# wjmaddox/online_gp

Hardware: AMD Instinct MI355X
Metric: streaming updates/sec (WISKI, 50^3 inducing grid) (higher is better)
Workload: dtype f32

## Files before the change

include/wiski.h:

```cpp
#ifndef WISKI_H
#define WISKI_H

#include <stdint.h>

#ifdef __cplusplus
extern "C" {
#endif

#define WISKI_OK 0
#define WISKI_E_BADARG (-1)
#define WISKI_E_LAUNCH (-2)
#define WISKI_E_WORKSPACE (-3)
#define WISKI_E_NOTCONV (-4)
#define WISKI_PENDING 1

#define WISKI_MAX_DIM 4

typedef struct wiski_grid {
  int32_t d;
  int32_t g[WISKI_MAX_DIM];
  double g0[WISKI_MAX_DIM];
  double h[WISKI_MAX_DIM];
} wiski_grid;

// ... 68 lines not shown
int64_t wiski_pcg_workspace_bytes(const wiski_grid* grid, int32_t k, int32_t max_iter, int32_t elem_size);
int wiski_pcg_f32(const wiski_grid* grid, const float* d_A_st, const float* d_tcol, float kscale, const float* d_evec, const float* d_evec2, const float* d_eval, float shift, const float* d_RHS, int32_t k, float* d_U, float* d_Z, int32_t warm, double tol, int32_t max_iter, int32_t check_every, int32_t first_check, void* d_work, int64_t work_bytes, int32_t* h_iters, double* h_relres, const int32_t* d_err, int32_t* h_err, int32_t a_sym, float* d_R, void* stream);
int wiski_pcg_f64(const wiski_grid* grid, const double* d_A_st, const double* d_tcol, double kscale, const double* d_evec, const double* d_evec2, const double* d_eval, double shift, const double* d_RHS, int32_t k, double* d_U, double* d_Z, int32_t warm, double tol, int32_t max_iter, int32_t check_every, int32_t first_check, void* d_work, int64_t work_bytes, int32_t* h_iters, double* h_relres, const int32_t* d_err, int32_t* h_err, int32_t a_sym, double* d_R, void* stream);

typedef int (*wiski_allreduce_fn)(void* ctx, void* d_vec, int64_t n_vec, int32_t elem_bytes, double* d_dots, int64_t n_dots, void* stream);
typedef struct wiski_shard {
  int32_t rank, nranks;
  void* comm;
  wiski_allreduce_fn allreduce;
  void* ctx;
} wiski_shard;
int wiski_shard_groups(int32_t d, int32_t rank, int32_t nranks, int32_t* g_lo, int32_t* g_hi);

typedef struct wiski_twolevel {
  int32_t r;
  int32_t nslab;
  const uint64_t* d_mask;
  const int32_t* d_off;
  const uint16_t* d_pos;
  const float* d_N;
  uint64_t* d_cs;
  float* d_mc;
  int32_t mc_cols;
} wiski_twolevel;

typedef struct wiski_pcg_async {
  int32_t state;
  int32_t it;
  int64_t seq;
  void* poll;
  int32_t prezeroed;
  int32_t guard_ok;
  double shift;
} wiski_pcg_async;
int wiski_pcg_async_f32(const wiski_grid* grid, const float* d_A_st, const float* d_tcol, float kscale, const float* d_evec, const float* d_evec2, const float* d_eval, float shift, const float* d_RHS, int32_t k, float* d_U, float* d_Z, int32_t warm, double tol, int32_t max_iter, int32_t check_every, int32_t first_check, void* d_work, int64_t work_bytes, int32_t* h_iters, double* h_relres, const int32_t* d_err, int32_t* h_err, int32_t a_sym, float* d_R, void* stream, wiski_pcg_async* handle, int32_t mode);
int wiski_pcg_async_f64(const wiski_grid* grid, const double* d_A_st, const double* d_tcol, double kscale, const double* d_evec, const double* d_evec2, const double* d_eval, double shift, const double* d_RHS, int32_t k, double* d_U, double* d_Z, int32_t warm, double tol, int32_t max_iter, int32_t check_every, int32_t first_check, void* d_work, int64_t work_bytes, int32_t* h_iters, double* h_relres, const int32_t* d_err, int32_t* h_err, int32_t a_sym, double* d_R, void* stream, wiski_pcg_async* handle, int32_t mode);
int wiski_pcg_async_free(wiski_pcg_async* handle);
int wiski_pcg_async_guard(const wiski_pcg_async* handle, const void** d_guard, int64_t* expect);
int wiski_pcg_zero_regions_f32(const wiski_grid* grid, int32_t k, int32_t max_iter, void* d_work, int32_t a_sym, void** p1, int64_t* n1_bytes, void** p2, int64_t* n2_bytes);
int wiski_pcg_zero_regions_f64(const wiski_grid* grid, int32_t k, int32_t max_iter, void* d_work, int32_t a_sym, void** p1, int64_t* n1_bytes, void** p2, int64_t* n2_bytes);
int64_t wiski_scatter_bin_bytes(const wiski_grid* grid, int64_t n, int32_t elem_size);
int wiski_scatter_stats_step_f32(const wiski_grid* grid, const float* d_x, const float* d_y, const float* d_wa, const float* d_wb, const float* d_noise, int64_t n, float* d_b, float* d_A_half, float* d_cnt, const float* d_u, float* d_res, float* d_mean_out, double* d_stats, int32_t* d_err, void* z1, int64_t n1_bytes, void* z2, int64_t n2_bytes, const void* d_guard, int64_t guard_expect, void* d_bin, int64_t bin_bytes, void* stream);
int wiski_scatter_stats_step_f64(const wiski_grid* grid, const double* d_x, const double* d_y, const double* d_wa, const double* d_wb, const double* d_noise, int64_t n, double* d_b, double* d_A_half, double* d_cnt, const double* d_u, double* d_res, double* d_mean_out, double* d_stats, int32_t* d_err, void* z1, int64_t n1_bytes, void* z2, int64_t n2_bytes, const void* d_guard, int64_t guard_expect, void* d_bin, int64_t bin_bytes, void* stream);
int wiski_gather_zero_f32(const wiski_grid* grid, const float* d_x, int64_t n, const float* d_V, int32_t k, float* d_out, int32_t* d_err, void* z1, int64_t n1_bytes, void* z2, int64_t n2_bytes, int32_t* zeroed, void* stream);
int wiski_gather_zero_f64(const wiski_grid* grid, const double* d_x, int64_t n, const double* d_V, int32_t k, double* d_out, int32_t* d_err, void* z1, int64_t n1_bytes, void* z2, int64_t n2_bytes, int32_t* zeroed, void* stream);

typedef struct wiski_stream_args_f32 {
  float* d_A_half; float* d_b; float* d_cnt; double* d_stats; int32_t* d_err;
  float* d_U; float* d_Z; float* d_R;
  const float* d_tcol; float kscale; const float* d_evec; const float* d_evec2; const float* d_eval; float shift;
  double tol; int32_t max_iter; int32_t check_every; void* d_work; int64_t work_bytes;
  void* d_bin; int64_t bin_bytes;
  const wiski_shard* shard;
  const wiski_twolevel* two_level;
  int32_t keep[3];
} wiski_stream_args_f32;
typedef struct wiski_stream_args_f64 {
  double* d_A_half; double* d_b; double* d_cnt; double* d_stats; int32_t* d_err;
  double* d_U; double* d_Z; double* d_R;
  const double* d_tcol; double kscale; const double* d_evec; const double* d_evec2; const double* d_eval; double shift;
  double tol; int32_t max_iter; int32_t check_every; void* d_work; int64_t work_bytes;
  void* d_bin; int64_t bin_bytes;
  const wiski_shard* shard;
  const wiski_twolevel* two_level;
  int32_t keep[3];
} wiski_stream_args_f64;
// ... 194 lines not shown
```

online_gp_amd/csrc/pcg.h:

```cpp
#pragma once
#include "wiski_common.h"

template <typename real>
struct PcgArgs {
  const real* A = nullptr;
  bool a_sym = false;
  const real* RHS = nullptr;
  int k = 0;
  const real* tcol = nullptr;
  real kscale = (real)0;
  const real* evec = nullptr;
  const real* evec2 = nullptr;
  const real* eval = nullptr;
  real shift = (real)0;
  const wiski_twolevel* two_level = nullptr;
  int keep[3] = {0, 0, 0};
  real* U = nullptr;
  real* Z = nullptr;
  real* R = nullptr;
  int warm = 0;
  double tol = 0;
  int max_iter = 0;
  int check_every = 0;
  int first_check = 0;
  void* work = nullptr;
  int64_t work_bytes = 0;
  int32_t* h_iters = nullptr;
  double* h_relres = nullptr;
  const int32_t* d_err = nullptr;
  int32_t* h_err = nullptr;
  wiski_pcg_async* handle = nullptr;
  int mode = 0;
  const wiski_shard* shard = nullptr;
};

template <typename real>
struct PcgLayout {
  static constexpr int SLOTS = 20;
  static int64_t align(int64_t v) { return (v + 255) / 256 * 256; }
  static int64_t bytes(int m, int k, int max_iter, int elem_size = (int)sizeof(real)) {
    return SLOTS * align((int64_t)k * m * elem_size) + align(PcgScal::doubles(k, max_iter) * 8);
  }
  real *r, *y, *p, *pt, *hp, *tmp;
  real* part;
  real* ty;
  real *sa, *sb;
  PcgScal S;
  int64_t km;
  int64_t nscal;
  PcgLayout(int m, int k, int max_iter, void* work) : km((int64_t)k * m), nscal(PcgScal::doubles(k, max_iter)) {
    char* w = static_cast<char*>(work);
    const int64_t vec = align(km * (int64_t)sizeof(real));
    auto at = [&](int slot) { return reinterpret_cast<real*>(w + slot * vec); };
    r = at(0); y = at(1); p = at(2); pt = at(3); hp = at(4); tmp = at(5); part = at(6); ty = at(14); sa = at(16); sb = at(18);
    double* base = reinterpret_cast<double*>(at(SLOTS));
    S = PcgScal{base, k, base + PcgScal::scalars(k, max_iter)};
  }
  double* zero1() const { return S.base; }
  int64_t zero1_count() const { return nscal; }
  real* zero2(int nch) const { return part + (int64_t)(nch > 0 ? nch - 1 : 0) * km; }
  int64_t zero2_count(int zl) const { return zl ? km : 0; }
};

// ... 7 lines not shown
```

online_gp_amd/csrc/solve.hip:

```cpp
#include "pcg.h"

#include <hip/hip_ext.h>

#include <chrono>
#include <cstdlib>
#include <map>
#include <mutex>
#include <vector>

static struct WiskiProf {
  bool on = false;
  bool armed = false;
  std::vector<hipEvent_t> ev;
  size_t used = 0;
  unsigned long long* d_stamp = nullptr;
  size_t stamp_pairs = 0, stamp_used = 0;
  struct Span { size_t off, n; };
  std::vector<Span> spans;
} g_prof;
constexpr unsigned long long PROF_CLOCK_MASK = 0xffffffffffffull;
constexpr size_t PROF_STAMP_ARENA_PAIRS = (size_t)1 << 20;

extern "C" int wiski_prof_start(int max_launches) {
  if (max_launches < 1) return WISKI_E_BADARG;
// ... 1334 lines not shown
  for (int q = 0; q < d; ++q) {
    if (G.g[q] > 128) return WISKI_E_BADARG;
    eoff[q + 1] = eoff[q] + G.g[q] * G.g[q];
  }
  dim3 grd((unsigned)((m + 255) / 256), (unsigned)k);
  const real* cur = d_V;
  for (int step = 0; step < 2 * d; ++step) {
    const int q = step < d ? step : step - d;
    const int transposed = step < d ? 1 : 0;
    real* dst = ((2 * d - 1 - step) % 2 == 0) ? d_out : d_tmp;
    const size_t sh = (size_t)G.g[q] * G.g[q] * sizeof(real);
    hipLaunchKernelGGL((k_dense_mode<real, 0>), grd, dim3(256), sh, s, G, q, d_evec + eoff[q], (const real*)nullptr, 0, transposed, cur, dst, (int64_t)0, d_eval, kscale,
                       shift, (const real*)nullptr, 0, (double*)nullptr);
    cur = dst;
    if (step == d - 1) hipLaunchKernelGGL((k_spectral_scale<real>), grd, dim3(256), 0, s, G, d_eval, kscale, shift, pw, rw, dst);
  }
  return hipGetLastError() == hipSuccess ? WISKI_OK : WISKI_E_LAUNCH;
}

struct WiskiPoll {
  double* h = nullptr;
  double* d = nullptr;
  long long* g = nullptr;
  int cap = 0;
  long long seq = 0;
};
static std::mutex g_poll_mu;
static std::map<int, WiskiPoll> g_polls;

static int poll_reserve(WiskiPoll& P, int k) {
  if (P.cap >= k) return WISKI_OK;
  if (P.h) (void)hipHostFree(P.h);
  const int cap = k < 64 ? 64 : k;
  if (hipHostMalloc((void**)&P.h, (size_t)(2 * cap + 3) * sizeof(double), hipHostMallocMapped | hipHostMallocCoherent | hipHostMallocPortable) !=
      hipSuccess)
    return WISKI_E_LAUNCH;
  if (hipHostGetDevicePointer((void**)&P.d, P.h, 0) != hipSuccess) return WISKI_E_LAUNCH;
  if (!P.g) {
    if (hipMalloc((void**)&P.g, sizeof(long long)) != hipSuccess) return WISKI_E_LAUNCH;
    if (hipMemset(P.g, 0, sizeof(long long)) != hipSuccess) return WISKI_E_LAUNCH;
  }
  P.h[0] = 0;
  P.cap = cap;
  return WISKI_OK;
}

#ifdef WISKI_STEP_TIMING
static double g_poll_wait_us = 0;
static long long g_poll_waits = 0, g_poll_waits_immediate = 0;
extern "C" void wiski_debug_poll_wait(double* us, long long* n, long long* immediate) {
  *us = g_poll_wait_us; *n = g_poll_waits; *immediate = g_poll_waits_immediate;
  g_poll_wait_us = 0; g_poll_waits = 0; g_poll_waits_immediate = 0;
}
struct PollWaitTimer {
  std::chrono::steady_clock::time_point t0 = std::chrono::steady_clock::now();
  bool immediate;
  explicit PollWaitTimer(bool imm) : immediate(imm) {}
  ~PollWaitTimer() {
    g_poll_wait_us += std::chrono::duration<double, std::micro>(std::chrono::steady_clock::now() - t0).count();
    ++g_poll_waits;
    if (immediate) ++g_poll_waits_immediate;
  }
};
#endif
static int poll_wait(WiskiPoll& P, long long seq, hipStream_t s) {
  volatile long long* flag = reinterpret_cast<volatile long long*>(P.h);
#ifdef WISKI_STEP_TIMING
// ... 3 lines not shown
  long spins = 0;
  while (__atomic_load_n(flag, __ATOMIC_ACQUIRE) != seq) {
    if ((++spins & 0xFFF) == 0 && std::chrono::steady_clock::now() - t0 > std::chrono::seconds(20)) {
      if (hipStreamSynchronize(s) != hipSuccess) return WISKI_E_LAUNCH;
      if (__atomic_load_n(flag, __ATOMIC_ACQUIRE) != seq) return WISKI_E_LAUNCH;
      break;
    }
  }
  return WISKI_OK;
}

__global__ void k_publish_flag(const int32_t* __restrict__ flag, double* __restrict__ poll, long long seq) {
  poll[1] = (double)*flag;
  __threadfence_system();
  __hip_atomic_store(reinterpret_cast<long long*>(poll), seq, __ATOMIC_RELEASE, __HIP_MEMORY_SCOPE_SYSTEM);
}

extern "C" int wiski_read_flag(const int32_t* d_flag, int32_t* h_value, void* stream) {
  if (!d_flag || !h_value) return WISKI_E_BADARG;
  int dev = 0;
  if (hipGetDevice(&dev) != hipSuccess) return WISKI_E_LAUNCH;
  std::lock_guard<std::mutex> lock(g_poll_mu);
  WiskiPoll& P = g_polls[dev];
  if (poll_reserve(P, 1) != WISKI_OK) return WISKI_E_LAUNCH;
  const long long seq = ++P.seq;
  hipStream_t s = (hipStream_t)stream;
  hipLaunchKernelGGL(k_publish_flag, dim3(1), dim3(1), 0, s, d_flag, P.d, seq);
  if (hipGetLastError() != hipSuccess) return WISKI_E_LAUNCH;
  if (int rc = poll_wait(P, seq, s)) return rc;
  *h_value = (int32_t)P.h[1];
  return WISKI_OK;
}

__global__ void k_pcg_publish(PcgScal S, int slot, double* __restrict__ poll, const int32_t* __restrict__ err, long long seq, double tol2,
                              long long* __restrict__ guard) {
  const int k = S.k;
  int ok = 1;
  for (int c = threadIdx.x; c < k; c += blockDim.x) {
    const double r0 = S.rn0()[c], r1 = S.rn(slot)[c];
    poll[1 + c] = r0;
    poll[1 + k + c] = r1;
    if (r0 > 0 && r1 > tol2 * r0) ok = 0;
  }
  ok = __syncthreads_and(ok);
  if (threadIdx.x == 0) {
    const double e = err ? (double)*err : 0.0;
    const long long gv = (ok && e == 0.0) ? seq : -seq;
    poll[1 + 2 * k] = e;
    poll[2 + 2 * k] = (double)gv;
    if (guard) *guard = gv;
  }
  __threadfence_system();
  __syncthreads();
  if (threadIdx.x == 0) __hip_atomic_store(reinterpret_cast<long long*>(poll), seq, __ATOMIC_RELEASE, __HIP_MEMORY_SCOPE_SYSTEM);
}

template <typename real>
__global__ __launch_bounds__(256) void k_pcg_zero(double* __restrict__ scal, int64_t nscal, real* __restrict__ vec, int64_t nvec) {
  const int64_t i = (int64_t)blockIdx.x * blockDim.x + threadIdx.x, stride = (int64_t)gridDim.x * blockDim.x;
  for (int64_t e = i; e < nscal; e += stride) scal[e] = 0.0;
  for (int64_t e = i; e < nvec; e += stride) vec[e] = (real)0;
}

template <typename real, int VEC>
__global__ __launch_bounds__(256) void k_pcg_init(int m, const real* __restrict__ rhs, const real* __restrict__ t, real* __restrict__ part,
                                                  int nch, int zl, int given, real* __restrict__ r, PcgScal S) {
  __shared__ double s_red[16];
  const int c = blockIdx.y;
  const int64_t km = (int64_t)S.k * m;
  double a = 0, bsum = 0;
  for (int i = (blockIdx.x * blockDim.x + threadIdx.x) * VEC; i < m; i += gridDim.x * blockDim.x * VEC) {
    const int64_t e = (int64_t)c * m + i;
    real f[VEC], rr[VEC];
    if constexpr (VEC == 4) {
      const Vec4<real> f4 = load4<real>(rhs + e);
      f[0] = f4.x; f[1] = f4.y; f[2] = f4.z; f[3] = f4.w;
      if (given) {
        const Vec4<real> r4 = load4<real>(r + e);
        rr[0] = r4.x; rr[1] = r4.y; rr[2] = r4.z; rr[3] = r4.w;
      } else {
      Vec4<real> t4;
      t4.x = t4.y = t4.z = t4.w = (real)0;
// ... 115 lines not shown
      } else {
        const Vec4<real> h4 = load4<real>(hp + e);
        hv[0] = h4.x; hv[1] = h4.y; hv[2] = h4.z; hv[3] = h4.w;
      }
    } else {
      pv[0] = p[e]; ptv[0] = pt[e]; uv[0] = u[e]; zv[0] = z[e]; rv[0] = r[e];
      if (nch > 0) {
        hv[0] = ptv[0];
        for (int ch = 0; ch < nch; ++ch) hv[0] += part[(int64_t)ch * km + e];
        if (zl) part[(int64_t)(nch - 1) * km + e] = (real)0;
      } else {
        hv[0] = hp[e];
      }
    }
#pragma unroll
    for (int q = 0; q < VEC; ++q) {
      uv[q] += al * pv[q];
      zv[q] += al * ptv[q];
      rv[q] -= al * hv[q];
      acc += (double)rv[q] * rv[q];
    }
    if constexpr (VEC == 4) {
      store4<real>(u + e, uv[0], uv[1], uv[2], uv[3]);
      store4<real>(z + e, zv[0], zv[1], zv[2], zv[3]);
      store4<real>(r + e, rv[0], rv[1], rv[2], rv[3]);
    } else {
      u[e] = uv[0]; z[e] = zv[0]; r[e] = rv[0];
    }
  }
  acc = block_reduce_sum(acc, s_red);
  if (poll == nullptr) {
    if (threadIdx.x == 0) unsafeAtomicAdd(S.rn(it + 1) + c, acc);
  } else {
    __shared__ int s_last;
    if (threadIdx.x == 0) {
      const double prev = atomicAdd(S.rn(it + 1) + c, acc);
      unsigned one = 1u;
      asm volatile("" : "+v"(one) : "v"(prev));
      const unsigned t = atomicAdd(S.ticket(), one);
      s_last = t == gridDim.x * gridDim.y - 1;
    }
    __syncthreads();
    if (s_last) {
      const int k = S.k;
      int ok = 1;
      for (int c2 = threadIdx.x; c2 < k; c2 += blockDim.x) {
        const double r0 = __hip_atomic_load(S.rn0() + c2, __ATOMIC_RELAXED, __HIP_MEMORY_SCOPE_AGENT);
        const double r1 = __hip_atomic_load(S.rn(it + 1) + c2, __ATOMIC_RELAXED, __HIP_MEMORY_SCOPE_AGENT);
        poll[1 + c2] = r0;
        poll[1 + k + c2] = r1;
        if (r0 > 0 && r1 > tol2 * r0) ok = 0;
      }
      ok = __syncthreads_and(ok);
      if (threadIdx.x == 0) {
        const double e = err ? (double)*err : 0.0;
        const long long gv = (ok && e == 0.0) ? seq : -seq;
        poll[1 + 2 * k] = e;
        poll[2 + 2 * k] = (double)gv;
        if (guard) *guard = gv;
        __hip_atomic_store(S.ticket(), 0u, __ATOMIC_RELAXED, __HIP_MEMORY_SCOPE_AGENT);
      }
      __threadfence_system();
      __syncthreads();
      if (threadIdx.x == 0) __hip_atomic_store(reinterpret_cast<long long*>(poll), seq, __ATOMIC_RELEASE, __HIP_MEMORY_SCOPE_SYSTEM);
    }
  }
}

template <typename real>
__global__ __launch_bounds__(256) void k_shard_reduce(int m4, int m, const real* __restrict__ part, int np, real* __restrict__ acc,
                                                      real* __restrict__ out) {
  for (int i = blockIdx.x * blockDim.x + threadIdx.x; i < m4; i += gridDim.x * blockDim.x) {
    Vec4<real> t = load4<real>(acc + 4 * i);
    for (int p = 0; p < np; ++p) {
      const Vec4<real> v = load4<real>(part + (int64_t)p * m + 4 * i);
      t.x += v.x; t.y += v.y; t.z += v.z; t.w += v.w;
    }
    store4<real>(out + 4 * i, t.x, t.y, t.z, t.w);
    store4<real>(acc + 4 * i, (real)0, (real)0, (real)0, (real)0);
  }
}


struct PcgPath {
  bool wide;
  bool sym;
  bool spectral;
  bool fused_cg;
  bool sharded;
  template <typename real>
  PcgPath(const GridDev<real>& G, const PcgArgs<real>& a)
      : wide(G.m % 4 == 0), sym(a.a_sym), spectral(a.evec != nullptr && a.eval != nullptr), fused_cg(spectral && wide && spectral_fused_ok<real>(G)),
        sharded(wiski_shard_active(a.shard)) {}
};

template <typename real>
static int pcg_validate(const GridDev<real>& G, const PcgArgs<real>& a, const PcgPath& path) {
  if (!a.A || !a.RHS || !a.U || !a.Z || !a.work || a.k < 1 || a.max_iter < 1) return WISKI_E_BADARG;
  if (a.mode != 0 && !a.handle) return WISKI_E_BADARG;
  if (a.mode == 2 && a.handle->state != 1) return WISKI_E_BADARG;
  if (!path.spectral && !a.tcol) return WISKI_E_BADARG;
  if (a.work_bytes < PcgLayout<real>::bytes(G.m, a.k, a.max_iter)) return WISKI_E_WORKSPACE;
  if (path.sharded) {
    if (!path.sym || !path.wide || a.k != 1 || a.shard->rank < 0 || a.shard->rank >= a.shard->nranks) return WISKI_E_BADARG;
    if (!a.shard->comm && !a.shard->allreduce) return WISKI_E_BADARG;
  }
  if (a.mode != 2 && a.warm == 2 && !a.R) return WISKI_E_BADARG;
  if (a.two_level && !(path.fused_cg && sizeof(real) == 4)) return WISKI_E_BADARG;
  if (a.keep[0] != 0 || a.keep[1] != 0 || a.keep[2] != 0) {
    if constexpr (sizeof(real) == 4) {
      if (!path.fused_cg || a.k != 1 || !spectral_keep_ok(G, a.keep, a.two_level != nullptr)) return WISKI_E_BADARG;
    } else {
      return WISKI_E_BADARG;
    }
  }
  return WISKI_OK;
}

template <typename real>
static int pcg_partials(const GridDev<real>& G, int k, bool sym, int* zl) {
  *zl = 0;
  if (G.m % 4 != 0) return 0;
  return sym ? sym_partials<real>(G, k, zl) : spmv_nch(G.d);
}

template <typename real>
struct PcgPlan {
  const GridDev<real>& G;
  const PcgArgs<real>& a;
  const PcgPath path;
  const hipStream_t s;
  const int m, k;
// ... 94 lines not shown
      if (int rc = plan.product(a.U, nullptr, (real)0, nullptr)) return rc;
      hipLaunchKernelGGL((k_pcg_init<real, 4>), plan.vgrid, dim3(256), 0, s, m, a.RHS, (const real*)a.Z, plan.cpart, plan.cnch, plan.czl, 0, plan.r, L.S);
    } else {
      if (int rc = plan.product(a.U, a.Z, (real)1, nullptr)) return rc;
      hipLaunchKernelGGL((k_pcg_init<real, 1>), plan.egrid, dim3(256), 0, s, m, a.RHS, (const real*)L.hp, (real*)nullptr, 0, 0, 0, plan.r, L.S);
    }
  } else {
    if (hipMemsetAsync(a.U, 0, (size_t)k * m * sizeof(real), s) != hipSuccess) return WISKI_E_LAUNCH;
    if (hipMemsetAsync(a.Z, 0, (size_t)k * m * sizeof(real), s) != hipSuccess) return WISKI_E_LAUNCH;
    hipLaunchKernelGGL((k_pcg_init<real, 1>), plan.egrid, dim3(256), 0, s, m, a.RHS, (const real*)nullptr, (real*)nullptr, 0, 0, 0, plan.r, L.S);
  }
  return WISKI_OK;
}

template <typename real>
static int pcg_iterate(const PcgPlan<real>& plan) {
  const GridDev<real>& G = plan.G;
  const PcgArgs<real>& a = plan.a;
  const PcgLayout<real>& L = plan.L;
  const PcgScal& S = L.S;
  const hipStream_t s = plan.s;
  const int m = plan.m, k = plan.k, max_iter = a.max_iter;
  const double tol2 = plan.tol2;
  const bool spectral = plan.path.spectral;
  real *const r = plan.r, *const p = L.p, *const pt = L.pt, *const hp = L.hp, *const cpart = plan.cpart;
  const int cnch = plan.cnch, czl = plan.czl;
  wiski_pcg_async* const as = a.handle;
  int mode = a.mode, first_check = a.first_check;
  const int check_every = a.check_every < 1 ? 10 : a.check_every;
  int rc = WISKI_OK;

  std::vector<double> h_rn0(k), h_rn(k);
  double err_seen = 0;
  int dev = 0;
  if (hipGetDevice(&dev) != hipSuccess) return WISKI_E_LAUNCH;
  std::unique_lock<std::mutex> poll_lock(g_poll_mu, std::defer_lock);
  WiskiPoll* Pp = nullptr;
  if (as) {
    if (!as->poll) as->poll = new WiskiPoll();
    Pp = static_cast<WiskiPoll*>(as->poll);
  } else {
    poll_lock.lock();
    Pp = &g_polls[dev];
  }
  WiskiPoll& P = *Pp;
  if (poll_reserve(P, k) != WISKI_OK) return WISKI_E_LAUNCH;
  auto collect = [&]() {
    for (int c = 0; c < k; ++c) {
      h_rn0[c] = P.h[1 + c];
      h_rn[c] = P.h[1 + k + c];
    }
    err_seen = P.h[1 + 2 * k];
  };
  bool deferred = false;
  auto fetch = [&](int slot, long long queued_seq = 0) -> int {
    long long seq = queued_seq;
    if (!seq) {
      seq = ++P.seq;
      hipLaunchKernelGGL(k_pcg_publish, dim3(1), dim3(64), 0, s, S, slot, P.d, a.d_err, seq, tol2, P.g);
    }
    if (hipGetLastError() != hipSuccess) return WISKI_E_LAUNCH;
    if (mode == 1) {
      as->state = 1;
      as->it = slot;
      as->seq = seq;
      deferred = true;
      return WISKI_OK;
    }
    if (int prc = poll_wait(P, seq, s)) return prc;
    collect();
    return WISKI_OK;
  };
  auto converged = [&]() {
    for (int c = 0; c < k; ++c)
      if (h_rn0[c] > 0 && h_rn[c] > tol2 * h_rn0[c]) return false;
    return true;
  };

  int it = 0;
  bool done = false;
  if (mode == 2) {
    it = as->it;
    as->state = 0;
    if (int prc = poll_wait(P, as->seq, s)) return prc;
    collect();
    as->guard_ok = (long long)P.h[2 + 2 * k] == as->seq ? 1 : 0;
    done = converged();
    first_check = it;
    mode = 0;
  }
  if (first_check < 1) first_check = check_every;
  if (first_check > max_iter) first_check = max_iter;
  auto due = [&](int i) { return i == max_iter || i == first_check || (i > first_check && (i - first_check) % check_every == 0); };
  bool pending = false;
  auto flush_update = [&](bool publish = false) -> long long {
    long long seq = 0;
    if (pending) {
      if (publish) seq = ++P.seq;
      hipLaunchKernelGGL((k_pcg_update_x<real, 4>), plan.vgrid, dim3(256), 0, s, m, it - 1, tol2, (const real*)p, (const real*)pt, (const real*)hp,
                         cpart, cnch, czl, a.U, a.Z, r, S, publish ? P.d : (double*)nullptr, a.d_err, seq, P.g);
      pending = false;
    }
    return seq;
  };
  while (!done && it < max_iter) {
    if (plan.path.fused_cg) {
      constexpr bool fuse_upd = sizeof(real) == 4;
      if (!fuse_upd) flush_update();
      const bool init_now = plan.init_in_fwd && it == 0;
      rc = launch_spectral_fused_cg<real>(G, a.evec, a.evec2, a.eval, a.kscale, a.shift, r, k, L.sa, L.sb, it, pending ? 1 : 0, tol2, p, pt, cpart, cnch,
                                          czl, a.U, a.Z, S, s, init_now ? a.RHS : (const real*)nullptr, a.two_level, a.keep);
      pending = false;
      if (rc) return rc;
      rc = plan.product_wide(p, pt, (real)1, S.php(it));
      if (rc) return rc;
      pending = true;
      ++it;
      if (due(it)) {
        rc = fetch(it, flush_update(true));
        if (rc) return rc;
        if (deferred) return WISKI_PENDING;
        done = converged();
      }
      continue;
    }
    if (spectral) {
      rc = launch_spectral_precond<real>(G, a.evec, a.evec2, a.eval, a.kscale, a.shift, r, k, L.sa, L.sb, L.ty, S.rho(it), s);
      if (rc) return rc;
      PCG_VEC_LAUNCH(plan, k_pcg_update_p, m, it, tol2, (const real*)(L.ty + (int64_t)k * m), (const real*)L.ty, p, pt, S);
    } else {
      rc = launch_kron<real>(G, a.tcol, r, k, a.kscale, L.tmp, L.y, r, S.rho(it), s);
      if (rc) return rc;
      PCG_VEC_LAUNCH(plan, k_pcg_update_p, m, it, tol2, (const real*)L.y, (const real*)r, p, pt, S);
    }
    rc = plan.product(p, pt, (real)1, S.php(it));
    if (rc) return rc;
    const bool pub = due(it + 1);
    const long long useq = pub ? ++P.seq : 0;
    PCG_VEC_LAUNCH(plan, k_pcg_update_x, m, it, tol2, (const real*)p, (const real*)pt, (const real*)hp, cpart, cnch, czl, a.U, a.Z, r, S,
                   pub ? P.d : (double*)nullptr, a.d_err, useq, P.g);
    ++it;
    if (due(it)) {
      rc = fetch(it, useq);
      if (rc) return rc;
      if (deferred) return WISKI_PENDING;
      done = converged();
    }
  }
  flush_update();
  if (hipGetLastError() != hipSuccess) return WISKI_E_LAUNCH;
  if (it == 0) {
    rc = fetch(0);
    if (rc) return rc;
  }
  if (a.h_iters) *a.h_iters = it;
  if (a.h_err) *a.h_err = (int32_t)err_seen;
  if (a.h_relres)
    for (int c = 0; c < k; ++c) a.h_relres[c] = h_rn0[c] > 0 ? sqrt(h_rn[c] / h_rn0[c]) : 0.0;
  return done ? WISKI_OK : WISKI_E_NOTCONV;
}
#undef PCG_VEC_LAUNCH

template <typename real>
int pcg(const wiski_grid* grid, const PcgArgs<real>& a, void* stream) {
  GridDev<real> G;
  int rc = make_grid_dev<real>(grid, &G);
  if (rc) return rc;
  const PcgPath path(G, a);
  rc = pcg_validate(G, a, path);
  if (rc) return rc;
  const PcgPlan<real> plan(G, a, path, (hipStream_t)stream);
  if (a.mode != 2) rc = pcg_start(plan);
  return rc ? rc : pcg_iterate(plan);
}
template int pcg<float>(const wiski_grid*, const PcgArgs<float>&, void*);
template int pcg<double>(const wiski_grid*, const PcgArgs<double>&, void*);

template <typename real>
static int spmv_impl(const wiski_grid* grid, const real* d_A, const real* d_V, int32_t k, const real* d_add, real beta, real* d_out, void* stream) {
  GridDev<real> G;
  int rc = make_grid_dev<real>(grid, &G);
  if (rc) return rc;
  if (!d_A || !d_V || !d_out || k < 1) return WISKI_E_BADARG;
  hipStream_t s = (hipStream_t)stream;
  if (G.m % 4 != 0) return launch_spmv<real>(G, d_A, d_V, k, d_add, beta, d_out, nullptr, s);
  const int nch = spmv_nch(G.d);
  const int64_t km = (int64_t)k * G.m;
  real* part = nullptr;
// ... 138 lines not shown
  if (int rc = make_grid_dev<float>(grid, &G)) return rc;
  if (!evec || !eval || !d_r || !w0 || !w1 || !d_y || !d_t || !d_rho || !keep || !spectral_fused_ok<float>(G) || G.m % 4) return WISKI_E_BADARG;
  const int kp[3] = {keep[0], keep[1], keep[2]};
  const bool any = kp[0] != 0 || kp[1] != 0 || kp[2] != 0;
  if (any && !spectral_keep_ok(G, kp, two_level != nullptr)) return WISKI_E_BADARG;
  PcgScal S{d_rho - 1, 1, nullptr};
  return launch_spectral_fused_cg<float>(G, evec, evec2, eval, kscale, shift, const_cast<float*>(d_r), 1, w0, w1, 0, 0, 0.0, d_y, d_t, (float*)nullptr, 0, 0,
                                         (float*)nullptr, (float*)nullptr, S, (hipStream_t)stream, (const float*)nullptr, two_level, any ? kp : (const int*)nullptr);
}
int wiski_precond_keep_ok(const wiski_grid* grid, const int32_t* keep, int32_t with_two_level) {
  GridDev<float> G;
  if (!keep || make_grid_dev<float>(grid, &G)) return 0;
  const int kp[3] = {keep[0], keep[1], keep[2]};
  return spectral_fused_ok<float>(G) && G.m % 4 == 0 && spectral_keep_ok(G, kp, with_two_level != 0) ? 1 : 0;
}
int wiski_shard_groups(int32_t d, int32_t rank, int32_t nranks, int32_t* g_lo, int32_t* g_hi) {
  if (d < 1 || d > WISKI_MAX_DIM || nranks < 1 || rank < 0 || rank >= nranks || !g_lo || !g_hi) return WISKI_E_BADARG;
  int lo, hi;
  shard_group_range(sym_groups(d), rank, nranks, &lo, &hi);
  *g_lo = lo;
  *g_hi = hi;
  return WISKI_OK;
}
int wiski_pcg_async_free(wiski_pcg_async* as) {
  if (!as) return WISKI_E_BADARG;
  if (as->poll) {
    WiskiPoll* P = static_cast<WiskiPoll*>(as->poll);
    if (P->h) (void)hipHostFree(P->h);
    if (P->g) (void)hipFree(P->g);
    delete P;
    as->poll = nullptr;
  }
  as->state = 0;
  return WISKI_OK;
}
int wiski_pcg_async_guard(const wiski_pcg_async* as, const void** d_guard, int64_t* expect) { return pcg_guard(as, d_guard, expect); }
int wiski_pcg_f32(const wiski_grid* g, PCG_ABI(float), void* s) { return pcg(g, pcg_args<float>(PCG_ABI_NAMES), s); }
int wiski_pcg_f64(const wiski_grid* g, PCG_ABI(double), void* s) { return pcg(g, pcg_args<double>(PCG_ABI_NAMES), s); }
}
```

online_gp_amd/csrc/stream_step.hip:

```cpp
#include "absorb.h"
#include "pcg.h"

template <typename real>
struct StreamArgs;
template <>
struct StreamArgs<float> { using type = wiski_stream_args_f32; };
template <>
struct StreamArgs<double> { using type = wiski_stream_args_f64; };

template <typename real>
static int absorb_batch(const wiski_grid* g, const typename StreamArgs<real>::type* a, AbsorbArgs<real> r, int carry, int zero, void* s) {
  r.b = a->d_b; r.A = a->d_A_half; r.half = true; r.cnt = a->d_cnt; r.stats = a->d_stats; r.err = a->d_err;
  r.u = carry || r.mean_out ? a->d_U : nullptr;
  r.res = carry ? a->d_R : nullptr;
  if (!r.mean_out) return absorb(g, r, s);
  if (zero) {
    if (int rc = pcg_zero_regions<real>(g, 1, a->max_iter, a->d_work, true, &r.z1, &r.n1_bytes, &r.z2, &r.n2_bytes)) return rc;
  }
  if (wiski_shard_active(a->shard)) {
    int32_t glo = 0, ghi = 0;
    if (int rc = wiski_shard_groups(g->d, a->shard->rank, a->shard->nranks, &glo, &ghi)) return rc;
    r.g_lo = glo; r.g_hi = ghi;
  } else {
    r.bin = a->d_bin; r.bin_bytes = a->bin_bytes;
  }
  return absorb(g, r, s);
}
template <typename real>
static PcgArgs<real> solve_args(const typename StreamArgs<real>::type* a, int carry, int first_check) {
  PcgArgs<real> p;
  p.A = a->d_A_half; p.a_sym = true; p.RHS = a->d_b; p.k = 1;
  p.tcol = a->d_tcol; p.kscale = a->kscale; p.evec = a->d_evec; p.evec2 = a->d_evec2; p.eval = a->d_eval; p.shift = a->shift; p.two_level = a->two_level;
  for (int q = 0; q < 3; ++q) p.keep[q] = a->keep[q];
  p.U = a->d_U; p.Z = a->d_Z; p.R = a->d_R; p.warm = carry ? 2 : 1;
  p.tol = a->tol; p.max_iter = a->max_iter; p.check_every = a->check_every; p.first_check = first_check;
  p.work = a->d_work; p.work_bytes = a->work_bytes;
  p.d_err = a->d_err;
  p.shard = a->shard;
  return p;
}

template <typename real>
static int stream_step_impl(const wiski_grid* grid, const typename StreamArgs<real>::type* a, const real* d_x, const real* d_y, const real* d_wa,
                            const real* d_wb, const real* d_noise, int64_t q, real* d_mean_out, int32_t carry, int32_t first_check, int32_t* h_iters,
                            double* h_relres, int32_t* h_err, void* stream, wiski_pcg_async* as, int32_t defer, int32_t* h_resumed) {
  if (!grid || !a || q < 0 || !a->d_A_half || !a->d_b || !a->d_U || !a->d_Z || !a->d_R) return WISKI_E_BADARG;
  if (q > 0 && (!d_x || !d_y || !d_wa || !d_wb || !d_noise)) return WISKI_E_BADARG;
  if (wiski_shard_active(a->shard) && q > 0 && !d_mean_out) return WISKI_E_BADARG;
  int rc = WISKI_OK;
  if (h_resumed) *h_resumed = 0;
  PcgArgs<real> solve = solve_args<real>(a, carry, first_check);
  solve.h_iters = h_iters; solve.h_relres = h_relres; solve.h_err = h_err; solve.handle = as;
  AbsorbArgs<real> batch;
  batch.x = d_x; batch.y = d_y; batch.wa = d_wa; batch.wb = d_wb; batch.noise = d_noise; batch.n = q; batch.mean_out = d_mean_out;
  bool absorbed = false;
  if (as && as->state == 1) {
    bool spec = false;
    if (q > 0 && d_mean_out) {
      const void* guard = nullptr;
      int64_t expect = 0;
      if (pcg_guard(as, &guard, &expect) == WISKI_OK) {
        AbsorbArgs<real> spec_batch = batch;
        spec_batch.guard = guard; spec_batch.guard_expect = expect;
        rc = absorb_batch<real>(grid, a, spec_batch, carry, 1, stream);
        if (rc) return rc;
        spec = true;
      }
    }
    {
      PcgArgs<real> resume = solve;
      resume.shift = (real)as->shift;
      resume.mode = 2;
      rc = pcg(grid, resume, stream);
    }
    if (h_resumed) *h_resumed = 1;
    if (rc != WISKI_OK && rc != WISKI_E_NOTCONV) return rc;
    absorbed = spec && as->guard_ok;
    if (q == 0) return rc;
    if (!absorbed && h_err && *h_err) return rc;
  } else if (q == 0 && as) {
    return WISKI_OK;
// ... 36 lines not shown
```

online_gp_amd/grid_ops.py:

```python
import ctypes
import math
import warnings

import numpy as np

import torch

from . import _hip


class GridSpec:

    def __init__(self, grid_bounds, grid_size):
        gb = [[float(lo), float(hi)] for lo, hi in (torch.as_tensor(grid_bounds, dtype=torch.float64).reshape(-1, 2).tolist())]
        d = len(gb)
        if not 1 <= d <= _hip.MAX_DIM:
            raise ValueError(f"grid dimension must be 1..{_hip.MAX_DIM}, got {d}")
        if isinstance(grid_size, int):
            g = [grid_size] * d
        else:
            g = [int(v) for v in grid_size]
        if len(g) != d:
            raise ValueError("grid_size / grid_bounds mismatch")
        if min(g) < 4:
            raise ValueError("cubic interpolation needs at least 4 grid points per dim")
        self.d = d
        self.g = g
        self.grid_bounds = gb
        delta = [(hi - lo) / (gi - 2) for (lo, hi), gi in zip(gb, g)]
        self.g0 = [lo - dl for (lo, hi), dl in zip(gb, delta)]
        self.h = [((hi + dl) - g0) / (gi - 1) for (lo, hi), dl, g0, gi in zip(gb, delta, self.g0, g)]
        from . import settings

        if settings.float32_grid.on():
# ... 849 lines not shown


class _Shard(ctypes.Structure):
    _fields_ = [("rank", ctypes.c_int32), ("nranks", ctypes.c_int32), ("comm", ctypes.c_void_p), ("allreduce", ALLREDUCE_FN), ("ctx", ctypes.c_void_p)]


class TwoLevelStruct(ctypes.Structure):
    _fields_ = [("r", ctypes.c_int32), ("nslab", ctypes.c_int32), ("d_mask", ctypes.c_void_p), ("d_off", ctypes.c_void_p), ("d_pos", ctypes.c_void_p),
                ("d_N", ctypes.c_void_p), ("d_cs", ctypes.c_void_p), ("d_mc", ctypes.c_void_p), ("mc_cols", ctypes.c_int32)]


def shard_groups(d, rank, nranks):
    lo, hi = ctypes.c_int32(0), ctypes.c_int32(0)
    _hip.check(_hip.lib().wiski_shard_groups(ctypes.c_int32(d), ctypes.c_int32(rank), ctypes.c_int32(nranks), ctypes.byref(lo), ctypes.byref(hi)),
               "wiski_shard_groups")
    return int(lo.value), int(hi.value)


def half_stencil_group_slices(grid, g_lo, g_hi):
    m = grid.m
    out = []
    for g in range(g_lo, g_hi):
        out.append((0, 4 * m) if g == 0 else ((7 * g - 3) * m, (7 * g + 4) * m))
    return out


class _StreamArgs64(ctypes.Structure):
    _fields_ = [(n, ctypes.c_double if t is ctypes.c_float else t) for n, t in _StreamArgs32._fields_]



class _PcgAsync(ctypes.Structure):
    _fields_ = [("state", ctypes.c_int32), ("it", ctypes.c_int32), ("seq", ctypes.c_int64), ("poll", ctypes.c_void_p),
                ("prezeroed", ctypes.c_int32), ("guard_ok", ctypes.c_int32), ("shift", ctypes.c_double)]


class StreamStep:

    def __init__(self, grid, dtype, device, A_half, b, cnt, stats, err, U, Z, R, tcol, workspace, max_iter):
        self.grid, self.dtype, self.device = grid, dtype, device
        self.keep = (A_half, b, cnt, stats, err, U, Z, R, tcol)
        self.args = (_StreamArgs32 if dtype == torch.float32 else _StreamArgs64)()
        a = self.args
        a.d_A_half, a.d_b, a.d_cnt, a.d_stats, a.d_err = A_half.data_ptr(), b.data_ptr(), cnt.data_ptr(), stats.data_ptr(), err.data_ptr()
        a.d_U, a.d_Z, a.d_R, a.d_tcol = U.data_ptr(), Z.data_ptr(), R.data_ptr(), tcol.data_ptr()
        buf, need = workspace.get(grid, 1, max_iter, dtype, device)
        self.keep += (buf,)
        a.d_work, a.work_bytes, a.max_iter = buf.data_ptr(), need, max_iter
        self.bin_buf = None
        self.fn = _hip.fn("wiski_stream_step", dtype)
        self.it, self.herr, self.rr = ctypes.c_int32(0), ctypes.c_int32(0), ctypes.c_double(0)
        self.eig_keep = None
        self.handle = _PcgAsync()
        self.resumed = ctypes.c_int32(0)

    @property
    def pending(self):
        return self.handle.state == 1

    def __del__(self):
        try:
            if self.handle.poll:
                _hip.lib().wiski_pcg_async_free(ctypes.byref(self.handle))
        except Exception:
            pass

    def set_shard(self, rank, nranks, comm=None, allreduce=None):
        if nranks < 1 or (nranks == 1 and not comm):
            self.args.shard = None
            self._shard = None
            return
        buf = self.keep[-1]
        base = buf.data_ptr()

        def cb(ctx, d_vec, n_vec, elem_bytes, d_dots, n_dots, stream):
            try:
                dt = torch.float32 if elem_bytes == 4 else torch.float64
                vec = buf[d_vec - base:d_vec - base + n_vec * elem_bytes].view(dt)
                dots = buf[d_dots - base:d_dots - base + n_dots * 8].view(torch.float64) if (d_dots and n_dots) else None
                allreduce(vec, dots)
                return 0
            except Exception:
                import traceback

                traceback.print_exc()
                return -2

# ... 8 lines not shown
    def set_keep(self, keep):
        k = tuple(int(v) for v in keep) if keep is not None else (0, 0, 0)
        if tuple(self.args.keep) != k:
            self.args.keep[:] = k

    def set_solver(self, kscale, eig, shift, tol, check_every):
        a = self.args
        evec, evals, evec2 = (tuple(eig) + (None,))[:3]
        self.eig_keep = (evec, evals, evec2)
        a.kscale, a.shift, a.tol, a.check_every = kscale, shift, tol, check_every
        a.d_evec, a.d_eval = evec.data_ptr(), evals.data_ptr()
        a.d_evec2 = evec2.data_ptr() if evec2 is not None else None

    def __call__(self, x, y, wa, wb, noise, mean_out, carry, first_check, defer=False):
        q = x.shape[0] if x is not None else 0
        if q >= 4096 and self.grid.d == 3 and (self.bin_buf is None or self.bin_q < q):
            f = _hip.lib().wiski_scatter_bin_bytes
            f.restype = ctypes.c_int64
            need = int(f(self.grid.ref, ctypes.c_int64(q), ctypes.c_int32(4 if self.dtype == torch.float32 else 8)))
            if need > 0:
                self.bin_buf, self.bin_q = torch.zeros(need, dtype=torch.uint8, device=self.device), q
                self.args.d_bin, self.args.bin_bytes = self.bin_buf.data_ptr(), need
        use_handle = defer or self.pending
        self.herr.value = 0
        rc = self.fn(self.grid.ref, ctypes.byref(self.args), _hip.dptr(x), _hip.dptr(y), _hip.dptr(wa), _hip.dptr(wb), _hip.dptr(noise),
                     ctypes.c_int64(q), _hip.dptr(mean_out), ctypes.c_int32(int(carry)), ctypes.c_int32(int(first_check)), ctypes.byref(self.it),
                     ctypes.byref(self.rr), ctypes.byref(self.herr), _hip.stream_ptr(self.device),
                     ctypes.byref(self.handle) if use_handle else None, ctypes.c_int32(int(defer)), ctypes.byref(self.resumed))
        if rc == -4:
            warnings.warn(f"wiski_pcg stopped at max_iter={self.args.max_iter} with relative residual {self.rr.value:.3e}", RuntimeWarning)
        elif rc != 1:
            _hip.check(rc, "wiski_stream_step")
        res = (int(self.it.value), float(self.rr.value), int(self.herr.value), rc != -4)
        if not use_handle:
            return res
        return (res if self.resumed.value == 1 else None), self.pending


def precond_apply(grid, eig, kscale, shift, r, two_level=None):
    Y, T, rho = precond_apply_cols(grid, eig, kscale, shift, r.reshape(1, grid.m), two_level=two_level)
    return Y.reshape(r.shape), T.reshape(r.shape), rho[0]


KEEP_EPS = 2.0 ** -30


def keep_counts(D_host, kscale, shift, eps=KEEP_EPS):
    import numpy as np

    if not (shift > 0 and kscale > 0):
        return None, 0.0, 0.0
    tau = eps / (1.0 - eps)
    dmax = [float(D[-1]) for D in D_host]
    if min(dmax) <= 0:
        return None, 0.0, 0.0
    K, lo, hi = [], 0.0, np.inf
    for q, D in enumerate(D_host):
        g = len(D)
        d = np.where(D < g * 2.0 ** -52 * dmax[q], 0.0, D)
        c = kscale * float(np.prod([dmax[p] for p in range(len(D_host)) if p != q]))
        first = int(np.searchsorted(d, tau / (shift * c), side="right"))
        K.append(g - first)
        if first < g:
            lo = max(lo, tau / (c * d[first]))
        if first > 0 and d[first - 1] > 0:
            hi = min(hi, tau / (c * d[first - 1]))
# ... 521 lines not shown
```

online_gp_amd/models/batched_fixed_noise_online_gp.py:

```python
import math

import torch

from .. import grid_ops, settings
from ..distributions import MultivariateNormal, ZeroLazyTensor, DenseLazyTensor, LazyCovariance
from ..kernels import GridInterpolationKernel, RBFKernel, ScaleKernel
from ..lazy.operators import (InducingPosterior, InterpolatedKernel, KroneckerToeplitz, PredictiveCovariance, StencilWtW, with_input_grad)
from ..lazy.dense_woodbury import DenseInducingPosterior
from ..likelihoods import FNMGLikelihood


class BatchOperator(LazyCovariance):

    def __init__(self, ops):
        self.ops = list(ops)
        self.shape = torch.Size([len(self.ops)]) + self.ops[0].shape
        self.dtype = self.ops[0].dtype
        self.device = self.ops[0].device

    def __getitem__(self, i):
        return self.ops[i]

    def __len__(self):
        return len(self.ops)
# ... 1513 lines not shown
            self._mean_state["R_ok"] = False
        self._give_up(cache)
        self._dump_caches()
        return self

    def stream_step(self, X, Y, want_mean=True):
        if self.grow_grid:
            self.grow_to_cover_(X)
        gamma = self._gamma()
        if gamma is not None:
            self._finish_pending()
        st = self._stream_fast_state(X, Y)
        if st is None:
            self._finish_pending()
            self.leave_stencil_shard()
            mean = None
            if want_mean:
                with settings.skip_posterior_variances(True):
                    mean = self(X).mean
            self.condition_on_observations(X, Y, None, inplace=True)
            self.prediction_cache
            return mean
        step, ms, pst = st
        if gamma is not None:
            self._decay(gamma, self.num_data, keep_mean_cache=True)
        q = X.shape[0]
        ones = self._ones(q)
        mean = torch.empty(q, dtype=self._dtype, device=self._device) if want_mean else None
        self._wsum_add(0, q, None)
        self.num_data = self.num_data + q
        self._refresh_count = getattr(self, "_refresh_count", 0) + 1
        self._two_level_step(step, pst, X, q)
        last = (getattr(self, "_last_iters", None) or [0])[0]
        fc, probe = self._first_poll(last)
        carry = ms.get("R_ok", False) and self._refresh_count % 16 != 0
        step.args.shift = float(self._wsum[0]) / pst["norm"]
        step.set_keep(self._keep_for_step(step, pst))
        y1 = Y.reshape(-1)
        y1 = y1 if y1.is_contiguous() else y1.contiguous()
        if "_spectral" in self.__dict__:
            self._spectral_absorb(0, X, None, y1)
        if settings.deferred_refresh.on() or step.pending:
            prev, pending = step(X, y1, ones, ones, ones, mean, carry, fc, defer=settings.deferred_refresh.on())
            if "path_probes" in self._kernel_cache and not (prev is not None and prev[2]):
                self._absorb_probes(self._kernel_cache, X, None)
            self._pending_step = step if pending else None
            if prev is not None:
                if prev[2]:
                    self._wsum_host[0] -= float(q)
                    self.num_data = self.num_data - q
                    self._refresh_count -= 1
                self._note_solve(ms, prev, *getattr(self, "_pending_fc", (0, False)))
            self._pending_fc = (fc, probe)
            if not pending:
                self._note_solve(ms, (step.it.value, step.rr.value, step.herr.value, True), fc, probe)
            return mean
        res = step(X, y1, ones, ones, ones, mean, carry, fc)
        if "path_probes" in self._kernel_cache:
            self._absorb_probes(self._kernel_cache, X, None)
        self._note_solve(ms, res, fc, probe)
        return mean

    def _keep_for_step(self, step, pst):
        if (settings.truncated_preconditioner.off() or self._dtype != torch.float32 or self._grid.d != 3 or self.num_outputs != 1
                or "eig_host" not in pst):
            return None
        kscale, shift = float(step.args.kscale), float(step.args.shift)
# ... 29 lines not shown
        if not self._two_level_applies():
            self.__dict__.pop("_two_level", None)
            return
        from ..lazy.two_level import TwoLevelTracker

        tr = self.__dict__.get("_two_level")
        if tr is None or init:
            if tr is None and not init:
                return
            tr = self.__dict__["_two_level"] = TwoLevelTracker()
        tr.note(X.reshape(-1, self._grid.d), wa)

    def _two_level_lose(self):
        tr = self.__dict__.get("_two_level")
        if tr is not None:
            tr.lose()

    def _two_level_step(self, step, pst, X, q):
        tr = self.__dict__.get("_two_level") if self._two_level_applies() else None
        tl = None
        if tr is not None:
            tr.note(X, None)
            _, s2, _ = self._hyper()[0]
            sh = self.__dict__.get("_stencil_shard")
            sub = max(settings.two_level_subsample.value(), sh["world"]) if sh is not None and sh["world"] > 1 else None
            tl = tr.for_step(self._grid, self._device, pst, 1.0 / s2, float(self._wsum[0]), self._err,
                             lockstep=sh is not None or settings.two_level_lockstep.on(),
                             last_iters=(getattr(self, "_last_iters", None) or [0])[0], subsample=sub)
            if tr.switched:
                self._poll_hint_sticky = 2
        if getattr(step, "_two_level", None) is not tl:
            step.set_two_level(tl)

    def _first_poll(self, last):
        if not last:
            return 0, False
        sticky = getattr(self, "_poll_hint_sticky", 0)
        if sticky:
            self._poll_hint_sticky = sticky - 1
            return min(last, 2), False
        hint = getattr(self, "_poll_hint", 0)
        if hint:
            return min(last, hint), False
        pend = getattr(self, "_probe_pending", 0)
        if pend:
            self._probe_pending = 0
            return pend, False
        wait = getattr(self, "_probe_wait", 0)
        rel = getattr(self, "_last_rel", None)
        tol = settings.cg_tolerance.value() or (1e-7 if self._dtype == torch.float32 else 1e-11)
        informed = rel is not None and rel < 0.1 * tol
        if informed:
            wait = min(wait, 4)
        probe = wait <= 0 and last > 1
        self._probe_informed = informed
        self._probe_wait = wait - 1
        fc = max(1, last - (1 if probe else 0))
        if probe:
            self._probe_pending = fc
        return fc, probe

    def _note_poll(self, it, fc, probe):
        if probe:
            self._probe_pending = 0
            if it <= fc:
                self._probe_gap, self._probe_wait = 0, 8
            elif getattr(self, "_probe_informed", False):
                self._probe_wait = 4
            else:
                self._probe_gap = min(32, max(8, 2 * getattr(self, "_probe_gap", 0)))
                self._probe_wait = self._probe_gap

    def _note_solve(self, ms, res, fc, probe=False):
        it, rel, flag, conv = res
        if fc:
            self._note_poll(it, fc, probe)
        self._last_iters = [it]
        self._last_rel = rel
        self._poll_hint = 0
        ms["R_ok"] = bool(conv)
        pc = self._memo.get("prediction_cache")
        if pc is not None:
            pc["cg_iters"] = [it]
        if flag:
            ms["R_ok"] = False
            self._raise_out_of_bounds(flag)

    def _finish_pending(self):
        step = self.__dict__.get("_pending_step")
        if step is None:
            return
        self._pending_step = None
        if step.pending:
            prev, _ = step(None, None, None, None, None, None, 0, 0, defer=False)
            if prev is not None and self._mean_state is not None:
                self._note_solve(self._mean_state, prev, *getattr(self, "_pending_fc", (0, False)))

    def _stream_fast_state(self, X, Y):
        if (self.robust_c is not None or self.window is not None or self._trend_deg is not None or self.num_outputs != 1 or self._use_dense() or settings.spectral_preconditioner.off() or settings.residual_carry_over.off()
                or X.dim() != 2 or not X.is_cuda or X.dtype != self._dtype or not X.is_contiguous() or Y.dtype != self._dtype):
            return None
        ms = self._mean_state
        pc = self._memo.get("prediction_cache")
        ver = self._hyper_version()
        if ms is None or pc is None or ms.get("ver") != ver or "pending_rank_update" in self._memo:
            return None
        op = _wtw_ops(self._kernel_cache["WtW"])[0]
        if not op.is_half or op.root is not None or "_cnt" not in self._kernel_cache:
# ... 413 lines not shown
```

online_gp_amd/settings.py:

```python


class _feature_flag:
    _state = False

    @classmethod
    def on(cls):
        return cls._state

    @classmethod
    def off(cls):
        return not cls._state

    @classmethod
    def _set_state(cls, state):
        cls._state = state

    def __init__(self, state=True):
        self.prev = self.__class__.on()
        self.state = state

    def __enter__(self):
        self.__class__._set_state(self.state)

    def __exit__(self, *args):
# ... 147 lines not shown


class two_level_rank(_value_context):

    _global_value = 192


class fused_factor_refresh(_feature_flag):

    _state = True


class two_level_rebuild(_feature_flag):

    _state = True


class two_level_min_iters(_value_context):

    _global_value = 4.0



class two_level_subsample(_value_context):

    _global_value = 1


class two_level_lockstep(_feature_flag):

    _state = False


class two_level_growth(_value_context):

    _global_value = 1.2


class two_level_lag(_value_context):

    _global_value = 2


class spectral_factor(_feature_flag):

    _state = True


class spectral_dense_regime(_feature_flag):

    _state = True


class spectral_tail(_value_context):

    _global_value = None


class spectral_mean_tolerance(_value_context):

    _global_value = None


class graphed_hyper_step(_feature_flag):

    _state = True
# ... 27 lines not shown
```

Before: 25.63 million.

## Use device-computed hindsight first-converged iteration to schedule first PCG poll

The publish kernels now scan up to 32 recent residual-norm slots per column and record, in the mapped host poll buffer, the earliest iteration at which every column met tolerance. The async handle stores this value, and a first_check of -1 makes the next solve place its first convergence poll there instead of relying on the Python-side sticky/probe heuristic. The aim is fewer host-device poll round trips and less wasted iteration past convergence. The cost is a small extra scan and shared atomic in the publish path, and a wrong hint could poll too early or too late. An optional per-step log file is also added.

```diff
diff --git a/include/wiski.h b/include/wiski.h
--- a/include/wiski.h
+++ b/include/wiski.h
@@ -124,6 +124,8 @@
   int32_t prezeroed;
   int32_t guard_ok;
   double shift;
+  int32_t first_ok;
+  int32_t first_ok_valid;
 } wiski_pcg_async;
 int wiski_pcg_async_f32(const wiski_grid* grid, const float* d_A_st, const float* d_tcol, float kscale, const float* d_evec, const float* d_evec2, const float* d_eval, float shift, const float* d_RHS, int32_t k, float* d_U, float* d_Z, int32_t warm, double tol, int32_t max_iter, int32_t check_every, int32_t first_check, void* d_work, int64_t work_bytes, int32_t* h_iters, double* h_relres, const int32_t* d_err, int32_t* h_err, int32_t a_sym, float* d_R, void* stream, wiski_pcg_async* handle, int32_t mode);
 int wiski_pcg_async_f64(const wiski_grid* grid, const double* d_A_st, const double* d_tcol, double kscale, const double* d_evec, const double* d_evec2, const double* d_eval, double shift, const double* d_RHS, int32_t k, double* d_U, double* d_Z, int32_t warm, double tol, int32_t max_iter, int32_t check_every, int32_t first_check, void* d_work, int64_t work_bytes, int32_t* h_iters, double* h_relres, const int32_t* d_err, int32_t* h_err, int32_t a_sym, double* d_R, void* stream, wiski_pcg_async* handle, int32_t mode);
diff --git a/online_gp_amd/csrc/pcg.h b/online_gp_amd/csrc/pcg.h
--- a/online_gp_amd/csrc/pcg.h
+++ b/online_gp_amd/csrc/pcg.h
@@ -29,6 +29,7 @@
   double* h_relres = nullptr;
   const int32_t* d_err = nullptr;
   int32_t* h_err = nullptr;
+  int32_t* h_first_ok = nullptr;
   wiski_pcg_async* handle = nullptr;
   int mode = 0;
   const wiski_shard* shard = nullptr;
diff --git a/online_gp_amd/csrc/solve.hip b/online_gp_amd/csrc/solve.hip
--- a/online_gp_amd/csrc/solve.hip
+++ b/online_gp_amd/csrc/solve.hip
@@ -1390,7 +1390,7 @@
   if (P.cap >= k) return WISKI_OK;
   if (P.h) (void)hipHostFree(P.h);
   const int cap = k < 64 ? 64 : k;
-  if (hipHostMalloc((void**)&P.h, (size_t)(2 * cap + 3) * sizeof(double), hipHostMallocMapped | hipHostMallocCoherent | hipHostMallocPortable) !=
+  if (hipHostMalloc((void**)&P.h, (size_t)(2 * cap + 4) * sizeof(double), hipHostMallocMapped | hipHostMallocCoherent | hipHostMallocPortable) !=
       hipSuccess)
     return WISKI_E_LAUNCH;
   if (hipHostGetDevicePointer((void**)&P.d, P.h, 0) != hipSuccess) return WISKI_E_LAUNCH;
@@ -1460,15 +1460,30 @@
   return WISKI_OK;
 }
 
+constexpr int PCG_NEVER_OK = 0x7fffffff;
+constexpr int PCG_HINDSIGHT_SLOTS = 32;
+__device__ __forceinline__ int pcg_first_ok(const PcgScal& S, int slot, int c, double r0, double tol2) {
+  if (!(r0 > 0)) return 0;
+  const double lim = tol2 * r0;
+  int first = PCG_NEVER_OK;
+  for (int j = slot, lo = slot > PCG_HINDSIGHT_SLOTS ? slot - PCG_HINDSIGHT_SLOTS : 0; j >= lo; --j)
+    if (__hip_atomic_load(S.rn(j) + c, __ATOMIC_RELAXED, __HIP_MEMORY_SCOPE_AGENT) <= lim) first = j;
+  return first;
+}
+
 __global__ void k_pcg_publish(PcgScal S, int slot, double* __restrict__ poll, const int32_t* __restrict__ err, long long seq, double tol2,
                               long long* __restrict__ guard) {
+  __shared__ int s_first;
   const int k = S.k;
   int ok = 1;
+  if (threadIdx.x == 0) s_first = 0;
+  __syncthreads();
   for (int c = threadIdx.x; c < k; c += blockDim.x) {
     const double r0 = S.rn0()[c], r1 = S.rn(slot)[c];
     poll[1 + c] = r0;
     poll[1 + k + c] = r1;
     if (r0 > 0 && r1 > tol2 * r0) ok = 0;
+    atomicMax(&s_first, pcg_first_ok(S, slot, c, r0, tol2));
   }
   ok = __syncthreads_and(ok);
   if (threadIdx.x == 0) {
@@ -1476,6 +1491,7 @@
     const long long gv = (ok && e == 0.0) ? seq : -seq;
     poll[1 + 2 * k] = e;
     poll[2 + 2 * k] = (double)gv;
+    poll[3 + 2 * k] = s_first == PCG_NEVER_OK ? -1.0 : (double)s_first;
     if (guard) *guard = gv;
   }
   __threadfence_system();
@@ -1657,13 +1673,14 @@
   if (poll == nullptr) {
     if (threadIdx.x == 0) unsafeAtomicAdd(S.rn(it + 1) + c, acc);
   } else {
-    __shared__ int s_last;
+    __shared__ int s_last, s_first;
     if (threadIdx.x == 0) {
       const double prev = atomicAdd(S.rn(it + 1) + c, acc);
       unsigned one = 1u;
       asm volatile("" : "+v"(one) : "v"(prev));
       const unsigned t = atomicAdd(S.ticket(), one);
       s_last = t == gridDim.x * gridDim.y - 1;
+      s_first = 0;
     }
     __syncthreads();
     if (s_last) {
@@ -1675,6 +1692,7 @@
         poll[1 + c2] = r0;
         poll[1 + k + c2] = r1;
         if (r0 > 0 && r1 > tol2 * r0) ok = 0;
+        atomicMax(&s_first, pcg_first_ok(S, it + 1, c2, r0, tol2));
       }
       ok = __syncthreads_and(ok);
       if (threadIdx.x == 0) {
@@ -1682,6 +1700,7 @@
         const long long gv = (ok && e == 0.0) ? seq : -seq;
         poll[1 + 2 * k] = e;
         poll[2 + 2 * k] = (double)gv;
+        poll[3 + 2 * k] = s_first == PCG_NEVER_OK ? -1.0 : (double)s_first;
         if (guard) *guard = gv;
         __hip_atomic_store(S.ticket(), 0u, __ATOMIC_RELAXED, __HIP_MEMORY_SCOPE_AGENT);
       }
@@ -1723,6 +1742,7 @@
 static int pcg_validate(const GridDev<real>& G, const PcgArgs<real>& a, const PcgPath& path) {
   if (!a.A || !a.RHS || !a.U || !a.Z || !a.work || a.k < 1 || a.max_iter < 1) return WISKI_E_BADARG;
   if (a.mode != 0 && !a.handle) return WISKI_E_BADARG;
+  if (a.first_check < -1 || (a.first_check == -1 && !a.handle)) return WISKI_E_BADARG;
   if (a.mode == 2 && a.handle->state != 1) return WISKI_E_BADARG;
   if (!path.spectral && !a.tcol) return WISKI_E_BADARG;
   if (a.work_bytes < PcgLayout<real>::bytes(G.m, a.k, a.max_iter)) return WISKI_E_WORKSPACE;
@@ -1883,6 +1903,7 @@
 
   std::vector<double> h_rn0(k), h_rn(k);
   double err_seen = 0;
+  int first_ok_seen = -1;
   int dev = 0;
   if (hipGetDevice(&dev) != hipSuccess) return WISKI_E_LAUNCH;
   std::unique_lock<std::mutex> poll_lock(g_poll_mu, std::defer_lock);
@@ -1902,6 +1923,7 @@
       h_rn[c] = P.h[1 + k + c];
     }
     err_seen = P.h[1 + 2 * k];
+    first_ok_seen = (int)P.h[3 + 2 * k];
   };
   bool deferred = false;
   auto fetch = [&](int slot, long long queued_seq = 0) -> int {
@@ -1940,6 +1962,7 @@
     first_check = it;
     mode = 0;
   }
+  if (first_check == -1) first_check = as->first_ok_valid ? (as->first_ok > 1 ? as->first_ok : 1) : 0;
   if (first_check < 1) first_check = check_every;
   if (first_check > max_iter) first_check = max_iter;
   auto due = [&](int i) { return i == max_iter || i == first_check || (i > first_check && (i - first_check) % check_every == 0); };
@@ -2005,6 +2028,11 @@
     if (rc) return rc;
   }
   if (a.h_iters) *a.h_iters = it;
+  if (a.h_first_ok) *a.h_first_ok = first_ok_seen;
+  if (as) {
+    as->first_ok = first_ok_seen;
+    as->first_ok_valid = first_ok_seen >= 0 ? 1 : 0;
+  }
   if (a.h_err) *a.h_err = (int32_t)err_seen;
   if (a.h_relres)
     for (int c = 0; c < k; ++c) a.h_relres[c] = h_rn0[c] > 0 ? sqrt(h_rn[c] / h_rn0[c]) : 0.0;
@@ -2209,6 +2237,8 @@
     as->poll = nullptr;
   }
   as->state = 0;
+  as->first_ok = 0;
+  as->first_ok_valid = 0;
   return WISKI_OK;
 }
 int wiski_pcg_async_guard(const wiski_pcg_async* as, const void** d_guard, int64_t* expect) { return pcg_guard(as, d_guard, expect); }
diff --git a/online_gp_amd/csrc/stream_step.hip b/online_gp_amd/csrc/stream_step.hip
--- a/online_gp_amd/csrc/stream_step.hip
+++ b/online_gp_amd/csrc/stream_step.hip
@@ -47,6 +47,7 @@
   if (!grid || !a || q < 0 || !a->d_A_half || !a->d_b || !a->d_U || !a->d_Z || !a->d_R) return WISKI_E_BADARG;
   if (q > 0 && (!d_x || !d_y || !d_wa || !d_wb || !d_noise)) return WISKI_E_BADARG;
   if (wiski_shard_active(a->shard) && q > 0 && !d_mean_out) return WISKI_E_BADARG;
+  if (first_check < -1 || (first_check == -1 && !as)) return WISKI_E_BADARG;
   int rc = WISKI_OK;
   if (h_resumed) *h_resumed = 0;
   PcgArgs<real> solve = solve_args<real>(a, carry, first_check);
diff --git a/online_gp_amd/grid_ops.py b/online_gp_amd/grid_ops.py
--- a/online_gp_amd/grid_ops.py
+++ b/online_gp_amd/grid_ops.py
@@ -1,5 +1,6 @@
 import ctypes
 import math
+import time
 import warnings
 
 import numpy as np
@@ -915,10 +916,13 @@
 
 class _PcgAsync(ctypes.Structure):
     _fields_ = [("state", ctypes.c_int32), ("it", ctypes.c_int32), ("seq", ctypes.c_int64), ("poll", ctypes.c_void_p),
-                ("prezeroed", ctypes.c_int32), ("guard_ok", ctypes.c_int32), ("shift", ctypes.c_double)]
+                ("prezeroed", ctypes.c_int32), ("guard_ok", ctypes.c_int32), ("shift", ctypes.c_double),
+                ("first_ok", ctypes.c_int32), ("first_ok_valid", ctypes.c_int32)]
 
 
 class StreamStep:
+
+    step_log = None
 
     def __init__(self, grid, dtype, device, A_half, b, cnt, stats, err, U, Z, R, tcol, workspace, max_iter):
         self.grid, self.dtype, self.device = grid, dtype, device
@@ -936,6 +940,7 @@
         self.eig_keep = None
         self.handle = _PcgAsync()
         self.resumed = ctypes.c_int32(0)
+        self.step_log = StreamStep.step_log
 
     @property
     def pending(self):
@@ -1010,6 +1015,12 @@
         elif rc != 1:
             _hip.check(rc, "wiski_stream_step")
         res = (int(self.it.value), float(self.rr.value), int(self.herr.value), rc != -4)
+        if self.step_log:
+            h = self.handle
+            with open(self.step_log, "a") as f:
+                f.write("t_us=%.1f q=%d first_check=%d placed=%d rc=%d resumed=%d iters=%d relres=%.3e guard_ok=%d first_ok=%d/%d\n" % (
+                    time.perf_counter() * 1e6, q, int(first_check), h.it if use_handle else -1, rc, self.resumed.value, res[0], res[1],
+                    h.guard_ok, h.first_ok, h.first_ok_valid))
         if not use_handle:
             return res
         return (res if self.resumed.value == 1 else None), self.pending
diff --git a/online_gp_amd/models/batched_fixed_noise_online_gp.py b/online_gp_amd/models/batched_fixed_noise_online_gp.py
--- a/online_gp_amd/models/batched_fixed_noise_online_gp.py
+++ b/online_gp_amd/models/batched_fixed_noise_online_gp.py
@@ -1569,7 +1569,9 @@
         self._refresh_count = getattr(self, "_refresh_count", 0) + 1
         self._two_level_step(step, pst, X, q)
         last = (getattr(self, "_last_iters", None) or [0])[0]
-        fc, probe = self._first_poll(last)
+        auto = (settings.poll_hindsight.on() and (settings.deferred_refresh.on() or step.pending)
+                and self.__dict__.get("_stencil_shard") is None and settings.two_level_lockstep.off())
+        fc, probe = self._first_poll(last, step.pending if auto else None)
         carry = ms.get("R_ok", False) and self._refresh_count % 16 != 0
         step.args.shift = float(self._wsum[0]) / pst["norm"]
         step.set_keep(self._keep_for_step(step, pst))
@@ -1665,9 +1667,13 @@
         if getattr(step, "_two_level", None) is not tl:
             step.set_two_level(tl)
 
-    def _first_poll(self, last):
+    def _first_poll(self, last, auto=None):
         if not last:
             return 0, False
+        if auto is not None:
+            self._poll_hint_sticky = self._probe_pending = 0
+            hint = getattr(self, "_poll_hint", 0)
+            return (min(last, hint) if hint and not auto else -1), False
         sticky = getattr(self, "_poll_hint_sticky", 0)
         if sticky:
             self._poll_hint_sticky = sticky - 1
@@ -1706,7 +1712,7 @@
 
     def _note_solve(self, ms, res, fc, probe=False):
         it, rel, flag, conv = res
-        if fc:
+        if fc > 0:
             self._note_poll(it, fc, probe)
         self._last_iters = [it]
         self._last_rel = rel
diff --git a/online_gp_amd/settings.py b/online_gp_amd/settings.py
--- a/online_gp_amd/settings.py
+++ b/online_gp_amd/settings.py
@@ -203,6 +203,11 @@
     _state = False
 
 
+class poll_hindsight(_feature_flag):
+
+    _state = True
+
+
 class two_level_growth(_value_context):
 
     _global_value = 1.2
```

Measured after the change: 26.08 million, median of 6. 1.02x the previous value.
